# martinmodrak/math

Hardware: AMD Instinct MI355X
Metric: gradient evals/sec (fp64), GP-marginal log-density N=4096 (higher is better)
Workload: dtype f64; 1 GPU; gp_marginal_gradient; N=4096, kernel=exp_quad, parallelism=replicas1

## Files before the change

### include/smg_hip.h

```cpp
#ifndef SMG_HIP_H
#define SMG_HIP_H

#include <stddef.h>

#ifdef __cplusplus
extern "C" {
#endif

enum smg_status_code {
  SMG_OK = 0,
  SMG_ERR_HIP = 1,
  SMG_ERR_NOT_PD = 2,
  SMG_ERR_NOT_SYMMETRIC = 4,
  SMG_ERR_NONFINITE = 8,
  SMG_ERR_ARG = 16,
  SMG_ERR_OOM = 32,
  SMG_ERR_NOT_POSITIVE = 64,
  SMG_ERR_SYNC = 128
};

typedef struct smg_ctx smg_ctx;

int smg_device_count(int* n_host);
int smg_ctx_create(int device, size_t initial_arena_bytes, smg_ctx** out_host);
int smg_ctx_destroy(smg_ctx* ctx);
int smg_ctx_device(const smg_ctx* ctx);
void* smg_ctx_stream(smg_ctx* ctx);

void* smg_arena_alloc(smg_ctx* ctx, size_t bytes);
size_t smg_arena_mark(smg_ctx* ctx);
int smg_arena_rewind(smg_ctx* ctx, size_t mark);
int smg_arena_recover_all(smg_ctx* ctx);
size_t smg_arena_used(const smg_ctx* ctx);
size_t smg_arena_reserved(const smg_ctx* ctx);
void* smg_host_scratch(smg_ctx* ctx, size_t bytes);
void* smg_pinned_io(smg_ctx* ctx, size_t bytes);
void* smg_pinned_result(smg_ctx* ctx, size_t bytes);
int smg_publish_to_host(smg_ctx* ctx, const double* src, long long n, double* dst);
int smg_gather_scalars(smg_ctx* ctx, const double* const* src, int n, double* dst, int* status_out);

int smg_memcpy_h2d(smg_ctx* ctx, void* dst, const void* src_host, size_t bytes);
int smg_memcpy_d2h(smg_ctx* ctx, void* dst_host, const void* src, size_t bytes);
int smg_memcpy_d2d(smg_ctx* ctx, void* dst, const void* src, size_t bytes);
int smg_memset(smg_ctx* ctx, void* dst, int value, size_t bytes);
int smg_memset_async(smg_ctx* ctx, void* dst, size_t bytes);
int smg_join_async(smg_ctx* ctx);
int smg_sync(smg_ctx* ctx);
int smg_sync_all(smg_ctx* ctx);
int smg_marker_record(smg_ctx* ctx, int slot);
int smg_marker_wait(smg_ctx* ctx, int slot);
int smg_status(smg_ctx* ctx, int* status_host);
int smg_status_armed(smg_ctx* ctx, int* armed);
int smg_status_enqueue(smg_ctx* ctx, int* host_dst);
int smg_status_inject(smg_ctx* ctx, int bits);
int smg_set_inv_block_mode(smg_ctx* ctx, int mode);
int smg_inv_block_fused(smg_ctx* ctx, int n);

enum smg_family {
  SMG_FAM_GEMM = 0, SMG_FAM_CHOL_FWD = 1, SMG_FAM_CHOL_REV = 2,
  SMG_FAM_GP = 3, SMG_FAM_MVN = 4, SMG_FAM_TRSV = 5, SMG_FAM_GLM = 6,
  SMG_FAM_ELEMWISE = 7,
  SMG_FAM_PANEL = 8,
  SMG_FAM_COMM = 9,
  SMG_FAM_COUNT = 10
};
int smg_profile_enable(smg_ctx* ctx, int on);
int smg_profile_read(smg_ctx* ctx, int family, double* total_ms_host, long long* count_host);
int smg_profile_flops(smg_ctx* ctx, int family, double* flops_host);

int smg_fill_unif(smg_ctx* ctx, double* out, long long n, unsigned long long seed,
                  double a, double b, double scale);
int smg_fill_bernoulli(smg_ctx* ctx, int* out, long long n, unsigned long long seed, double p);

int smg_gemm(smg_ctx* ctx, int transA, int transB, int uplo, int m, int n, int k,
             double alpha, const double* A, int lda, const double* B, int ldb,
             double beta, double* C, int ldc);
#define SMG_TRI_A_LOWER 1
#define SMG_TRI_A_UPPER 2
#define SMG_TRI_B_LOWER 4
#define SMG_TRI_B_UPPER 8
int smg_gemm_tri(smg_ctx* ctx, int transA, int transB, int uplo, int tri, int m, int n, int k, double alpha,
                 const double* A, int lda, const double* B, int ldb, double beta, double* C, int ldc);


int smg_gp_exp_quad_cov_fwd(smg_ctx* ctx, const double* x, int n, double sigma,
                            double l, double* K, int ldk);
int smg_gp_exp_quad_cov_rev(smg_ctx* ctx, const double* x, int n, double sigma,
                            double l, const double* Kadj, int ldka, double* out2);

int smg_gp_exp_quad_cov_nd_fwd(smg_ctx* ctx, const double* x, int D, int n, double sigma,
                               double l, double* K, int ldk);
int smg_gp_exp_quad_cov_nd_rev(smg_ctx* ctx, const double* x, int D, int n, double sigma,
                               double l, const double* Kadj, int ldka, double* out2);

enum smg_gp_family { SMG_GP_EXP_QUAD = 0, SMG_GP_EXPONENTIAL = 1, SMG_GP_MATERN32 = 2, SMG_GP_MATERN52 = 3 };
int smg_gp_cov_fwd(smg_ctx* ctx, int family, const double* x, int D, int n, double sigma, double l,
                   double* K, int ldk);
int smg_gp_cov_rev(smg_ctx* ctx, int family, const double* x, int D, int n, double sigma, double l,
                   const double* Kadj, int ldka, double* out2);

int smg_gp_exp_quad_cov_tangent_fwd(smg_ctx* ctx, const double* x, int n, double sigma,
                                    double l, double dsigma, double dl, double* Kd, int ldk);
int smg_gp_exp_quad_cov_tangent_rev(smg_ctx* ctx, const double* x, int n, double sigma,
                                    double l, double dsigma, double dl, const double* Kdadj,
                                    int ldka, double* out4);

int smg_add_diag_fwd(smg_ctx* ctx, const double* A, int lda, int n,
                     double d_scalar, const double* d_vec, double* B, int ldb);
int smg_add_diag_rev(smg_ctx* ctx, const double* Badj, int ldb, int n,
                     double* Aadj, int ldaa, double* dadj, int d_is_vec);

long long smg_cholesky_aux_doubles(int n);
int smg_cholesky_block_size(int n);
int smg_check_symmetric(smg_ctx* ctx, const double* A, int lda, int n);
int smg_cholesky_fwd(smg_ctx* ctx, const double* A, int lda, int n, double* L,
// ... 228 lines not shown
```

### math_amd/csrc/ctx.hip

```cpp
#include <cstdio>
#include <cstdlib>
#include <cstring>

#include "smg_internal.h"

namespace {

constexpr size_t kAlign = 256;

__global__ void k_reduce_partials(const double* __restrict__ p, int nparts,
                                  int width, double* out, int accumulate) {
  __shared__ double lds[16];
  const int c = blockIdx.x;
  double s = 0.0;
  for (int i = threadIdx.x; i < nparts; i += blockDim.x) s += p[(size_t)i * width + c];
  s = block_sum(s, lds);
  if (threadIdx.x == 0) out[c] = accumulate ? out[c] + s : s;
}

__global__ __launch_bounds__(256) void k_publish(const double* __restrict__ src, long long n, double* dst,
                                                 long long* done, long long seq) {
  for (long long i = threadIdx.x; i < n; i += blockDim.x)
    __hip_atomic_store(dst + i, src[i], __ATOMIC_RELAXED, __HIP_MEMORY_SCOPE_SYSTEM);
  asm volatile("s_waitcnt vmcnt(0)" ::: "memory");
// ... 198 lines not shown
  ctx->side = nullptr;
  ctx->main_stream = nullptr;
  for (int i = 0; i < SMG_FAM_COUNT; ++i) {
    ctx->prof_ms[i] = 0;
    ctx->prof_count[i] = 0;
    ctx->prof_flops[i] = 0;
  }
  int prio_least = 0, prio_greatest = 0;
  if (hipDeviceGetStreamPriorityRange(&prio_least, &prio_greatest) != hipSuccess) prio_greatest = 0;
  if (hipStreamCreateWithPriority(&ctx->stream, hipStreamNonBlocking, prio_greatest) != hipSuccess) {
    delete ctx;
    return SMG_ERR_HIP;
  }
  if (initial < (size_t)(64u << 20)) initial = (size_t)(64u << 20);
  char* base = nullptr;
  if (hipMalloc(&base, initial) != hipSuccess) {
    hipStreamDestroy(ctx->stream);
    delete ctx;
    return SMG_ERR_OOM;
  }
  ctx->blocks.push_back({base, initial});
  if (hipMalloc(&ctx->status_d, SMG_STATUS_BYTES) != hipSuccess ||
      hipHostMalloc(&ctx->status_h, 256, hipHostMallocDefault) != hipSuccess) {
    delete ctx;
    return SMG_ERR_HIP;
  }
  hipMemset(ctx->status_d, 0, SMG_STATUS_BYTES);
  ctx->flags_d = ctx->status_d + 64;
  ctx->flag_epoch = 0;
  ctx->inv_ctr_d = reinterpret_cast<unsigned*>(ctx->flags_d + 4096);
  ctx->inv_launches = 0;
  ctx->inv_per_cu = ctx->inv_cus = -1;
  ctx->inv_mode = 0;
  ctx->host_scratch_size = 1u << 20;
  if (hipHostMalloc(&ctx->host_scratch, ctx->host_scratch_size, hipHostMallocDefault) != hipSuccess) {
    delete ctx;
    return SMG_ERR_HIP;
  }
  if (hipHostMalloc(&ctx->done_h, 256, hipHostMallocCoherent | hipHostMallocMapped) != hipSuccess ||
      hipMalloc(&ctx->red_counter_d, 256) != hipSuccess) {
    delete ctx;
    return SMG_ERR_HIP;
  }
  *(volatile long long*)ctx->done_h = 0;
  hipMemset(ctx->red_counter_d, 0, 256);
  hipDeviceSynchronize();
  *out = ctx;
  return SMG_OK;
}

int smg_ctx_destroy(smg_ctx* ctx) {
  if (!ctx) return SMG_OK;
  hipSetDevice(ctx->device);
  hipStreamSynchronize(ctx->stream);
  prof_drain(ctx);
  smg_comm_destroy(ctx);
  for (auto& b : ctx->blocks) hipFree(b.base);
  for (auto e : ctx->prof_pool) hipEventDestroy(e);
  for (auto e : ctx->ev_pool) hipEventDestroy(e);
  for (auto e : ctx->ev_fork) hipEventDestroy(e);
  for (auto e : ctx->marker_ev) hipEventDestroy(e);
  if (ctx->status_ev) hipEventDestroy(ctx->status_ev);
  if (ctx->zero_stream) {
    hipStreamSynchronize(ctx->zero_stream);
    hipEventDestroy(ctx->zero_ev_main);
    hipEventDestroy(ctx->zero_ev_done);
// ... 324 lines not shown
int smg_join_async(smg_ctx* ctx) {
  if (!ctx) return SMG_ERR_ARG;
  if (ctx->inv_pending) {
    SMG_HIP_TRY(hipStreamWaitEvent(ctx->stream, ctx->inv_ev, 0));
    ctx->inv_pending = 0;
  }
  if (int e = smg_zero_flush(ctx)) return e;
  if (!ctx->zero_pending) return SMG_OK;
  SMG_HIP_TRY(hipStreamWaitEvent(ctx->stream, ctx->zero_ev_done, 0));
  ctx->zero_pending = 0;
  return SMG_OK;
}

int smg_marker_record(smg_ctx* ctx, int slot) {
  if (!ctx) return SMG_ERR_ARG;
  hipEvent_t e;
  if (int rc = smg_marker_event(ctx, slot, &e)) return rc;
  SMG_HIP_TRY(hipEventRecord(e, ctx->stream));
  return SMG_OK;
}

int smg_marker_wait(smg_ctx* ctx, int slot) {
  if (!ctx || slot < 0 || slot >= (int)ctx->marker_ev.size()) return SMG_ERR_ARG;
  SMG_HIP_TRY(hipEventSynchronize(ctx->marker_ev[slot]));
  return SMG_OK;
}

int smg_set_inv_block_mode(smg_ctx* ctx, int mode) {
  if (!ctx || mode < 0 || mode > 1) return SMG_ERR_ARG;
  ctx->inv_mode = mode;
  return SMG_OK;
}

int smg_sync_all(smg_ctx* ctx) {
  if (!ctx) return SMG_ERR_ARG;
  sync_all_streams(ctx);
  SMG_HIP_TRY(hipGetLastError());
  if (ctx->prof_on) prof_drain(ctx);
  return SMG_OK;
}

int smg_sync(smg_ctx* ctx) {
  SMG_HIP_TRY(hipStreamSynchronize(ctx->stream));
  if (ctx->prof_on) prof_drain(ctx);
  return SMG_OK;
}

int smg_status(smg_ctx* ctx, int* status) {
  hipLaunchKernelGGL(k_status_take, dim3(1), dim3(64), 0, ctx->stream, ctx->status_d, ctx->status_h);
  SMG_LAUNCH_CHECK();
  SMG_HIP_TRY(hipStreamSynchronize(ctx->stream));
  if (ctx->prof_on) prof_drain(ctx);
  int s = ctx->status_h[0] | ctx->host_status;
  ctx->host_status = 0;
  ctx->status_armed = 0;
  if (status) *status = s;
  return SMG_OK;
}

}

int smg_status_mark_impl(smg_ctx* ctx) {
  if (!ctx->status_ev && hipEventCreateWithFlags(&ctx->status_ev, hipEventDisableTiming) != hipSuccess) {
    ctx->status_ev = nullptr;
    return SMG_ERR_HIP;
  }
// ... 127 lines not shown
```

### math_amd/csrc/gemm.hip

```cpp
#include "smg_internal.h"
#include <cstdio>
#include <cstdlib>
#include <type_traits>

#ifndef SMG_GEMM_TRI128_MIN
#define SMG_GEMM_TRI128_MIN 1024
#endif
#ifndef SMG_GEMM_KS2_MAX
#define SMG_GEMM_KS2_MAX 1536
#endif
#ifndef SMG_GEMM_NR64
#define SMG_GEMM_NR64 2
#endif
#ifndef SMG_GEMM_NR32
#define SMG_GEMM_NR32 2
#endif

namespace {

template <int BM, int BK, bool KCONTIG>
struct lds_layout;
template <int BM, int BK>
struct lds_layout<BM, BK, false> {
  static_assert(BM % 32 == 0, "BM");
  static constexpr int size = BK * BM;
  __device__ static int at(int i, int kk) { return kk * BM + (i ^ ((kk & 1) << 4)); }
};
template <int BM, int BK>
struct lds_layout<BM, BK, true> {
  static_assert(BK == 16 || BK == 32, "BK");
  static constexpr int size = BM * BK;
  __device__ static int at(int i, int kk) {
    return i * BK + (kk ^ (BK == 16 ? (i & 14) : ((i & 15) << 1)));
  }
};

template <int I, int N, typename F>
__device__ __forceinline__ void smg_static_for_impl(F&& f) {
  if constexpr (I < N) {
    f(std::integral_constant<int, I>{});
    smg_static_for_impl<I + 1, N>(f);
  }
}
template <int N, typename F>
__device__ __forceinline__ void smg_static_for(F&& f) {
  smg_static_for_impl<0, N>(f);
}

__device__ double g_gemm_zero[2] = {0.0, 0.0};

template <int BM, int BK, bool KCONTIG, int NT = 256>
__device__ __forceinline__ void load_tile(const double* __restrict__ X, int ld,
                                          int rows, int k, int i0, int k0,
                                          double (&r)[BM * BK / NT]) {
  constexpr int PER = BM * BK / NT;
#pragma unroll
  for (int q = 0; q < PER; ++q) {
    const int e = threadIdx.x + NT * q;
    int i, kk;
    if (KCONTIG) {
      i = e / BK;
      kk = e % BK;
    } else {
      kk = e / BM;
      i = e % BM;
    }
    const int gi = i0 + i, gk = k0 + kk;
    const double* p = KCONTIG ? X + ((size_t)gi * ld + gk) : X + (gi + (size_t)gk * ld);
// ... 18 lines not shown
    lds[lds_layout<BM, BK, KCONTIG>::at(i, kk)] = r[q];
  }
}

__device__ __forceinline__ void tri_decode(int t, int& bi, int& bj) {
  int r = (int)((sqrt(8.0 * (double)t + 1.0) - 1.0) * 0.5);
  while ((r + 1) * (r + 2) / 2 <= t) ++r;
  while (r * (r + 1) / 2 > t) --r;
  bi = r;
  bj = t - r * (r + 1) / 2;
}

__device__ __forceinline__ void tri_decode_grouped(int t, int T, int& bi, int& bj) {
  constexpr int G = 8;
  int r, c;
  tri_decode(t, r, c);
  const int r0 = r / G * G, r1 = min(r0 + G, T), h = r1 - r0;
  int q = t - r0 * (r0 + 1) / 2;
  if (q < r0 * h) {
    bi = r0 + q % h;
    bj = q / h;
    return;
  }
  q -= r0 * h;
  int j = r0;
  while (q >= r1 - j) {
    q -= r1 - j;
    ++j;
  }
  bi = j + q;
  bj = j;
}

template <int BM, int BN, int BK, bool TA, bool TB, int MODE, int KS = 1>
__global__ __launch_bounds__(256 * KS) void k_gemm(
    int m, int n, int k, double alpha, const double* __restrict__ A, int lda,
    const double* __restrict__ B, int ldb, double beta, double* __restrict__ C,
    int ldc, int tiles_m, int ntiles, int kchunk, double* __restrict__ slab, long long sA,
    long long sB, long long sC, int px, int ntp, int tri, double* __restrict__ C2, int ldc2, int bz) {
  constexpr bool LOWT = MODE == 1 || MODE == 3;
  constexpr bool UPT = MODE == 2;
  constexpr bool TRIC = LOWT || UPT;
  A += blockIdx.y * sA;
  B += blockIdx.y * sB;
  C += blockIdx.y * sC;
  constexpr bool AK = TA;
  constexpr bool BKC = !TB;
  using LA = lds_layout<BM, BK, AK>;
  using LB = lds_layout<BN, BK, BKC>;
  constexpr int NR = BM == 128 ? 1 : (BM == 64 ? SMG_GEMM_NR64 : SMG_GEMM_NR32);
  constexpr int STAGE = LA::size + LB::size;
  constexpr int OPS = 2 * STAGE;
  constexpr int ECH = (BM * BN + BN <= OPS) ? BN : 32;
  constexpr int POOL = (OPS > (BM + 1) * ECH) ? OPS : (BM + 1) * ECH;
  __shared__ double pool[POOL];

  int bi, bj, tile, split;
  const bool tri_a_only = !TRIC && (tri & 3) && !(tri & 12);
  const bool tri_b_only = !TRIC && (tri & 12) && !(tri & 3);
  if (px > 0) {
    split = blockIdx.x / ntp;
    const int tb = blockIdx.x - split * ntp;
    const int x = tb & 7, l = tb >> 3, py = 8 / px;
    const int tiles_n = ntiles / tiles_m;
    const int rx = x % px, ry = x / px;
    const int r0 = rx * tiles_m / px, r1 = (rx + 1) * tiles_m / px;
    const int c0 = ry * tiles_n / py, c1 = (ry + 1) * tiles_n / py;
    const int rm = r1 - r0;
    if (rm <= 0 || l >= rm * (c1 - c0)) return;
    tile = (r0 + l % rm) + (c0 + l / rm) * tiles_m;
  } else {
    tile = blockIdx.x % ntiles;
    split = blockIdx.x / ntiles;
  }
  const bool tri_sq = TRIC && m == n && BM == BN;
  if (LOWT && tri_sq) {
    const int T = tiles_m;
    int r, q;
    if (tri == SMG_TRI_B_LOWER) {
      tri_decode(ntiles - 1 - tile, r, q);
      bj = T - 1 - r;
      bi = bj + q;
    } else if (tri == SMG_TRI_B_UPPER || tri == (SMG_TRI_A_LOWER | SMG_TRI_B_UPPER)) {
      tri_decode(tile, r, q);
      bj = T - 1 - r;
// ... 32 lines not shown
  if (tri) {
    int lo = 0, hi = k;
    if (tri & 1) hi = min(hi, i0 + BM);
    if (tri & 2) lo = max(lo, i0);
    if (tri & 4) lo = max(lo, j0);
    if (tri & 8) hi = min(hi, j0 + BN);
    lo = lo / BK * BK;
    kbeg = max(kbeg, lo);
    kend = min(kend, hi);
    if (kend < kbeg) kend = kbeg;
  }

  constexpr int TM = BM / 32, TN = BN / 32;
  constexpr int NT = 256 * KS;
  const int lane = threadIdx.x & 63, wave = threadIdx.x >> 6;
  const int wr = (wave & 3) >> 1, wc = wave & 1, kg = KS == 1 ? 0 : wave >> 2;
  d4 acc[TM][TN];
#pragma unroll
  for (int a = 0; a < TM; ++a)
#pragma unroll
    for (int b = 0; b < TN; ++b) acc[a][b] = d4{0.0, 0.0, 0.0, 0.0};

  constexpr int PA = BM * BK / NT, PB = BN * BK / NT;
  double ra[NR][PA], rb[NR][PB];
  const int nst = (kend - kbeg + BK - 1) / BK;
  auto gload = [&](int set, int st) {
    load_tile<BM, BK, AK, NT>(A, lda, m, kend, i0, kbeg + st * BK, ra[set]);
    load_tile<BN, BK, BKC, NT>(B, ldb, n, kend, j0, kbeg + st * BK, rb[set]);
  };
  auto lstore = [&](int set, int buf) {
    store_tile<BM, BK, AK, NT>(pool + buf * STAGE, ra[set]);
    store_tile<BN, BK, BKC, NT>(pool + buf * STAGE + LA::size, rb[set]);
  };
#pragma unroll
  for (int j = 0; j < NR; ++j) gload(j, j);
  constexpr int EPT = BM * BN / NT;
  constexpr bool PREFETCH_C = EPT <= 16;
  const bool use_c = !slab && beta != 0.0 && !(bz > 0 && i0 >= bz) && !(bz < 0 && j0 >= -bz);
  double cpre[PREFETCH_C ? EPT : 1];
  if (PREFETCH_C) {
#pragma unroll
    for (int q = 0; q < EPT; ++q) {
      const int e = threadIdx.x + NT * q;
      const int i = i0 + e % BM, j = j0 + e / BM;
      cpre[q] = (use_c && i < m && j < n) ? C[i + (size_t)j * ldc] : 0.0;
    }
  }
  const int fr = lane & 15, fk = lane >> 4;
  static_assert(BK / 4 % KS == 0, "K stage split");
  auto mma_stage = [&](const double* Ab, const double* Bb) {
#pragma unroll
    for (int kq = 0; kq < BK / 4 / KS; ++kq) {
      const int ks = kg * (BK / 4 / KS) + kq;
      double af[TM], bf[TN];
#pragma unroll
      for (int a = 0; a < TM; ++a)
        af[a] = Ab[LA::at(wr * (BM / 2) + a * 16 + fr, ks * 4 + fk)];
#pragma unroll
      for (int b = 0; b < TN; ++b)
        bf[b] = Bb[LB::at(wc * (BN / 2) + b * 16 + fr, ks * 4 + fk)];
#pragma unroll
      for (int a = 0; a < TM; ++a)
#pragma unroll
        for (int b = 0; b < TN; ++b)
          acc[a][b] = __builtin_amdgcn_mfma_f64_16x16x4f64(af[a], bf[b], acc[a][b], 0, 0, 0);
    }
  };
  lstore(0, 0);
  gload(0, NR);
  __syncthreads();
  constexpr int U = NR % 2 == 0 ? NR : 2 * NR;
  auto body = [&](int st, auto uc) {
    constexpr int u = decltype(uc)::value;
    mma_stage(pool + (u & 1) * STAGE, pool + (u & 1) * STAGE + LA::size);
    lstore((u + 1) % NR, (u & 1) ^ 1);
    gload((u + 1) % NR, st + 1 + NR);
    __syncthreads();
  };
  int s0 = 0;
  for (; s0 + U <= nst; s0 += U)
    smg_static_for<U>([&](auto uc) { body(s0 + decltype(uc)::value, uc); });
  smg_static_for<U - 1>([&](auto uc) {
    if (s0 + decltype(uc)::value < nst) body(s0 + decltype(uc)::value, uc);
  });

  __syncthreads();
#pragma unroll
  for (int c0 = 0; c0 < BN; c0 += ECH) {
#pragma unroll
    for (int g = 0; g < KS; ++g) {
      if (kg == g) {
#pragma unroll
        for (int a = 0; a < TM; ++a)
#pragma unroll
          for (int b = 0; b < TN; ++b) {
            const int jl = wc * (BN / 2) + b * 16 + (lane & 15) - c0;
            if (jl < 0 || jl >= ECH) continue;
#pragma unroll
            for (int r = 0; r < 4; ++r) {
              double* d = &pool[jl * (BM + 1) + wr * (BM / 2) + a * 16 + (lane >> 4) + 4 * r];
              *d = g == 0 ? acc[a][b][r] : *d + acc[a][b][r];
            }
          }
      }
      __syncthreads();
    }
#pragma unroll
    for (int q = 0; q < BM * ECH / NT; ++q) {
      const int e = threadIdx.x + NT * q;
      const int il = e % BM, jl = e / BM;
      const int i = i0 + il, j = j0 + c0 + jl;
      if (i >= m || j >= n) continue;
      if (LOWT && i < j) {
        if (MODE == 3 && C2) C2[i + (size_t)j * ldc2] = 0.0;
        continue;
      }
      if (UPT && i > j) continue;
// ... 38 lines not shown
                                                        double alpha, double beta, double* __restrict__ C, int ldc,
                                                        int lower, int bz) {
  const long long tot = (long long)m * n;
  for (smg_mn w(m >> 1, n); w.ok(); w.next()) {
    const int i = 2 * w.i, j = w.j;
    if (lower == 1 && i + 1 < j) continue;
    if (lower == 2 && i > j) continue;
    const long long e = (long long)j * m + i;
    d2v s = {0.0, 0.0};
    int t = 0;
    for (; t + 4 <= splits; t += 4) {
      const d2v a0 = *reinterpret_cast<const d2v*>(slab + (size_t)t * tot + e);
      const d2v a1 = *reinterpret_cast<const d2v*>(slab + (size_t)(t + 1) * tot + e);
      const d2v a2 = *reinterpret_cast<const d2v*>(slab + (size_t)(t + 2) * tot + e);
      const d2v a3 = *reinterpret_cast<const d2v*>(slab + (size_t)(t + 3) * tot + e);
      s += a0;
      s += a1;
      s += a2;
      s += a3;
    }
    for (; t < splits; ++t) s += *reinterpret_cast<const d2v*>(slab + (size_t)t * tot + e);
    double* c = C + i + (size_t)j * ldc;
    const bool w0 = !(lower == 1 && i < j), w1 = !(lower == 2 && i + 1 > j);
    const double b = ((bz > 0 && i >= bz) || (bz < 0 && j >= -bz)) ? 0.0 : beta;
    if (w0) c[0] = (b == 0.0) ? alpha * s[0] : alpha * s[0] + b * c[0];
    if (w1) c[1] = (b == 0.0) ? alpha * s[1] : alpha * s[1] + b * c[1];
  }
}

thread_local double* t_c2 = nullptr;
thread_local int t_ldc2 = 0;
thread_local int t_bz = 0;

template <int BM, int BN, int BK, bool TA, bool TB, int MODE, int KS = 1>
int launch(smg_ctx* ctx, int m, int n, int k, double alpha, const double* A,
           int lda, const double* B, int ldb, double beta, double* C, int ldc, int batch = 1,
           long long sA = 0, long long sB = 0, long long sC = 0, int tri = 0) {
  constexpr bool TRIC = MODE == 1 || MODE == 2 || MODE == 3;
  const int tm = smg_ceil_div(m, BM), tn = smg_ceil_div(n, BN);
  const int ntiles = (TRIC && m == n && BM == BN) ? tm * (tm + 1) / 2 : tm * tn;
  int splits = 1;
  const int target = 512;
  constexpr int KMIN = 64;
  const bool covers = ntiles >= 256 && k <= 1024;
  if (!tri && MODE != 3 && MODE != 4 && batch == 1 && ntiles < target && !covers &&
      k >= 2 * KMIN) {
    splits = smg_ceil_div(target, ntiles);
    const int maxs = k / KMIN;
    if (splits > maxs) splits = maxs;
    if (splits > 64) splits = 64;
    if (splits < 1) splits = 1;
  }
  int kchunk = smg_ceil_div(smg_ceil_div(k, splits), BK) * BK;
  splits = smg_ceil_div(k, kchunk);
  double* slab = nullptr;
  if (splits > 1) {
    const int slot = ctx->stream == ctx->side                                ? SMG_WS_GEMM_SIDE
                     : (ctx->zero_stream && ctx->stream == ctx->zero_stream) ? SMG_WS_GEMM_ZERO
                                                                             : SMG_WS_GEMM;
    slab = smg_ws(ctx, slot, (size_t)splits * m * n);
    if (!slab) return SMG_ERR_OOM;
  }
  const bool tri_one = !TRIC && tri && (!(tri & 3) || !(tri & 12));
  int px = 0, ntp = ntiles;
  if (!(TRIC && m == n && BM == BN) && ntiles >= 64 && !tri_one) {
    long long best = -1;
    for (int p = 1; p <= 8; p *= 2) {
      const int q = 8 / p;
      if (p > tm || q > tn) continue;
      const long long rr = smg_ceil_div(tm, p), cc = smg_ceil_div(tn, q);
      const long long foot = rr * BM + cc * BN;
      if (best < 0 || foot < best) {
        best = foot;
        px = p;
        ntp = 8 * (int)(rr * cc);
      }
    }
  }
  hipLaunchKernelGGL((k_gemm<BM, BN, BK, TA, TB, MODE, KS>), dim3(ntp * splits, batch), dim3(256 * KS), 0,
                     ctx->stream, m, n, k, alpha, A, lda, B, ldb, beta, C, ldc, tm,
                     ntiles, kchunk, slab, sA, sB, sC, px, ntp, tri, MODE >= 3 ? t_c2 : nullptr,
                     MODE >= 3 ? t_ldc2 : 0, t_bz);
  if (splits > 1) {
    const long long tot = (long long)m * n;
    if ((m & 1) == 0) {
      const long long pairs = tot / 2;
      const int nb = (int)(pairs / 256 < 2048 ? (pairs + 255) / 256 : 2048);
      hipLaunchKernelGGL(k_splitk_reduce2, dim3(nb), dim3(256), 0, ctx->stream, m, n, splits, slab, alpha, beta,
                         C, ldc, MODE, t_bz);
    } else {
      hipLaunchKernelGGL(k_splitk_reduce, dim3(smg_ceil_div(tot, 256)), dim3(256), 0,
                         ctx->stream, m, n, splits, slab, alpha, beta, C, ldc, MODE, t_bz);
    }
  }
  SMG_LAUNCH_CHECK();
  return SMG_OK;
}

inline bool overlaps(const double* X, int ldx, int rows, int cols, const double* C, int ldc, int m,
                     int n) {
  if (rows <= 0 || cols <= 0 || m <= 0 || n <= 0) return false;
  const double* x1 = X + (size_t)(cols - 1) * ldx + rows;
  const double* c1 = C + (size_t)(n - 1) * ldc + m;
  if (!(X < c1 && C < x1)) return false;
  if (ldx != ldc) return true;
  const double* base = X < C ? X : C;
  const long long ox = X - base, oc = C - base, ld = ldx;
  const long long rx = ox % ld, cx = ox / ld, rc = oc % ld, cc = oc / ld;
  return rx < rc + m && rc < rx + rows && cx < cc + n && cc < cx + cols;
}

constexpr int BK64 = 16;

template <bool TA, bool TB, int MODE>
int dispatch_tile(smg_ctx* ctx, int m, int n, int k, double alpha, const double* A,
                  int lda, const double* B, int ldb, double beta, double* C, int ldc, int tri) {
  constexpr bool FULLC = MODE == 0 || MODE == 4;
  const bool alias_a = overlaps(A, lda, TA ? k : m, TA ? m : k, C, ldc, m, n);
  const bool alias_b = overlaps(B, ldb, TB ? n : k, TB ? k : n, C, ldc, m, n);
  if (alias_a || alias_b) {
    if (MODE == 3 || MODE == 4 || t_bz) return SMG_ERR_ARG;
    if (MODE == 0 && alias_a && !alias_b && n <= 64)
      return launch<32, 64, 32, TA, TB, 0>(ctx, m, n, k, alpha, A, lda, B, ldb, beta, C, ldc, 1, 0, 0, 0, tri);
    if (MODE == 0 && alias_b && !alias_a && m <= 64)
      return launch<64, 32, 32, TA, TB, 0>(ctx, m, n, k, alpha, A, lda, B, ldb, beta, C, ldc, 1, 0, 0, 0, tri);
    double* T = smg_ws(ctx, SMG_WS_ALIAS, (size_t)m * n);
    if (!T) return SMG_ERR_OOM;
    int rc = dispatch_tile<TA, TB, MODE>(ctx, m, n, k, alpha, A, lda, B, ldb, 0.0, T, m, tri);
    if (rc) return rc;
    if (beta == 0.0) return smg_copy_impl(ctx, m, n, T, m, C, ldc, 1.0, 0);
    if (beta != 1.0) {
      rc = smg_scale_impl(ctx, m, n, beta, C, ldc, MODE);
      if (rc) return rc;
    }
    return smg_copy_impl(ctx, m, n, T, m, C, ldc, 1.0, 1);
  }
  const long long big_tiles = (long long)smg_ceil_div(m, 128) * smg_ceil_div(n, 128);
  const long long t64 = smg_ceil_div(m, 64);
  const long long mid_tiles =
      (!FULLC && m == n) ? t64 * (t64 + 1) / 2 : t64 * smg_ceil_div(n, 64);
  if (FULLC && big_tiles >= (tri ? SMG_GEMM_TRI128_MIN : 256) && k > 128)
    return launch<128, 128, 16, TA, TB, MODE>(ctx, m, n, k, alpha, A, lda, B, ldb, beta, C, ldc, 1, 0, 0, 0, tri);
  if (MODE == 0 && TA && !TB && k >= 1536 && mid_tiles < 512)
    return launch<128, 64, 16, TA, TB, MODE>(ctx, m, n, k, alpha, A, lda, B, ldb, beta, C, ldc, 1, 0, 0, 0, tri);
  if (mid_tiles >= 512) {
    if (mid_tiles <= SMG_GEMM_KS2_MAX)
      return launch<64, 64, BK64, TA, TB, MODE, 2>(ctx, m, n, k, alpha, A, lda, B, ldb, beta, C, ldc, 1, 0, 0, 0, tri);
    return launch<64, 64, BK64, TA, TB, MODE>(ctx, m, n, k, alpha, A, lda, B, ldb, beta, C, ldc, 1, 0, 0, 0, tri);
  }
  const bool tall_nn = MODE == 0 && !TA && !TB && n <= 512;
  if (mid_tiles >= 256 && !tall_nn)
    return launch<64, 64, BK64, TA, TB, MODE, 2>(ctx, m, n, k, alpha, A, lda, B, ldb, beta, C, ldc, 1, 0, 0, 0, tri);
  const long long t32 = smg_ceil_div(m, 32);
  const long long small_tiles = (!FULLC && m == n) ? t32 * (t32 + 1) / 2 : t32 * smg_ceil_div(n, 32);
  if (small_tiles <= 256)
    return launch<32, 32, 32, TA, TB, MODE, 2>(ctx, m, n, k, alpha, A, lda, B, ldb, beta, C, ldc, 1, 0, 0, 0, tri);
  return launch<32, 32, 32, TA, TB, MODE>(ctx, m, n, k, alpha, A, lda, B, ldb, beta, C, ldc, 1, 0, 0, 0, tri);
}

}

int smg_gemm_batched_impl(smg_ctx* ctx, int ta, int tb, int m, int n, int k, double alpha,
                          const double* A, int lda, long long sA, const double* B, int ldb,
                          long long sB, double beta, double* C, int ldc, long long sC, int batch) {
  if (m <= 0 || n <= 0 || batch <= 0) return SMG_OK;
  if (k <= 0 || alpha == 0.0) return SMG_ERR_ARG;
  smg_prof_scope prof(ctx, SMG_FAM_GEMM);
  if (ctx->prof_on) ctx->prof_flops[SMG_FAM_GEMM] += 2.0 * m * n * k * batch;
  const bool big = (long long)smg_ceil_div(m, 64) * smg_ceil_div(n, 64) * batch >= 192;
#define SMG_BATCHED(TA_, TB_)                                                                    \
  return big ? launch<64, 64, BK64, TA_, TB_, 0>(ctx, m, n, k, alpha, A, lda, B, ldb, beta, C, ldc, \
                                               batch, sA, sB, sC)                                 \
             : launch<32, 32, 32, TA_, TB_, 0>(ctx, m, n, k, alpha, A, lda, B, ldb, beta, C, ldc, \
// ... 71 lines not shown

int smg_gemm_sym_phi_impl(smg_ctx* ctx, int ta, int tb, int n, int k, double alpha, const double* A, int lda,
                          const double* B, int ldb, double beta, double* C, int ldc, double* P, int ldp, int tri) {
  if (n <= 0) return SMG_OK;
  if (k <= 0 || alpha == 0.0 || !P) return SMG_ERR_ARG;
  smg_prof_scope prof(ctx, SMG_FAM_GEMM);
  if (ctx->prof_on) {
    const double cut = (tri & 3) && (tri & 12) ? 1.0 / 3.0 : (tri ? 0.5 : 1.0);
    ctx->prof_flops[SMG_FAM_GEMM] += cut * 2.0 * k * ((double)n * n - (double)n * (n - 1) / 2);
  }
  t_c2 = P;
  t_ldc2 = ldp;
  int rc;
  if (!ta && !tb) rc = dispatch_tile<false, false, 3>(ctx, n, n, k, alpha, A, lda, B, ldb, beta, C, ldc, tri);
  else if (ta && !tb) rc = dispatch_tile<true, false, 3>(ctx, n, n, k, alpha, A, lda, B, ldb, beta, C, ldc, tri);
  else if (!ta && tb) rc = dispatch_tile<false, true, 3>(ctx, n, n, k, alpha, A, lda, B, ldb, beta, C, ldc, tri);
  else rc = dispatch_tile<true, true, 3>(ctx, n, n, k, alpha, A, lda, B, ldb, beta, C, ldc, tri);
  t_c2 = nullptr;
  return rc;
}

extern "C" int smg_gemm_tri(smg_ctx* ctx, int ta, int tb, int uplo, int tri, int m, int n, int k,
                            double alpha, const double* A, int lda, const double* B, int ldb, double beta,
                            double* C, int ldc) {
  if (!ctx || m < 0 || n < 0 || k < 0 || tri < 0 || tri > 15) return SMG_ERR_ARG;
  if ((m > 0 && n > 0) && (!C || ldc < m)) return SMG_ERR_ARG;
  if (k > 0 && m > 0 && n > 0 && alpha != 0.0) {
    if (!A || !B) return SMG_ERR_ARG;
    if (lda < (ta ? k : m) || ldb < (tb ? n : k)) return SMG_ERR_ARG;
  }
  return smg_gemm_impl(ctx, ta, tb, uplo, m, n, k, alpha, A, lda, B, ldb, beta, C, ldc, tri);
}

extern "C" int smg_gemm(smg_ctx* ctx, int ta, int tb, int uplo, int m, int n, int k,
                        double alpha, const double* A, int lda, const double* B,
                        int ldb, double beta, double* C, int ldc) {
  if (!ctx || m < 0 || n < 0 || k < 0) return SMG_ERR_ARG;
  if ((m > 0 && n > 0) && (!C || ldc < m)) return SMG_ERR_ARG;
  if (k > 0 && m > 0 && n > 0 && alpha != 0.0) {
    if (!A || !B) return SMG_ERR_ARG;
    if (lda < (ta ? k : m) || ldb < (tb ? n : k)) return SMG_ERR_ARG;
  }
  return smg_gemm_impl(ctx, ta, tb, uplo, m, n, k, alpha, A, lda, B, ldb, beta, C, ldc);
}
```

### math_amd/csrc/smg_internal.h

```cpp
#pragma once
#include <hip/hip_runtime.h>

#include <cstddef>
#include <cstdint>
#include <utility>
#include <vector>

#include "../../include/smg_hip.h"

typedef double d4 __attribute__((ext_vector_type(4)));
typedef double d2v __attribute__((ext_vector_type(2)));

struct smg_arena_block {
  char* base;
  size_t size;
};

struct smg_prof_slot {
  hipEvent_t start, stop;
  int family;
};

constexpr int SMG_INV_CTRS = 64;
constexpr size_t SMG_STATUS_BYTES = 256 + 4096 * sizeof(int) + SMG_INV_CTRS * sizeof(int);

struct smg_ctx {
  int device;
  hipStream_t stream;
  hipStream_t side;
  hipStream_t main_stream;
  std::vector<hipEvent_t> ev_pool;
  std::vector<hipEvent_t> ev_fork;
  std::vector<hipEvent_t> marker_ev;
  std::vector<smg_arena_block> blocks;
  size_t cur_block;
  size_t offset;
  int* status_d;
  int* status_h;
  int host_status;
  int status_armed;
  hipEvent_t status_ev;
  int status_mark;
  hipStream_t zero_stream;
  hipStream_t copy_stream;
  hipEvent_t zero_ev_main, zero_ev_done;
  int zero_pending;
  std::vector<std::pair<void*, size_t>> zero_queue;
  hipEvent_t inv_ev, inv_ev_main, inv_ev_aux;
  int inv_pending;
  hipEvent_t inv_ev_w;
  int inv_w_recorded;
  int* flags_d;
  int flag_epoch;
  unsigned* inv_ctr_d;
  long long inv_launches;
  int inv_per_cu, inv_cus;
  int inv_mode;
  void* host_scratch;
  size_t host_scratch_size;
  void* pin_io;
  size_t pin_io_size;
  void* res_h;
  size_t res_h_size;
  long long* done_h;
  long long done_seq;
  unsigned int* red_counter_d;
  double* ws[12];
  size_t ws_doubles[12];
  int prof_on;
  std::vector<smg_prof_slot> prof_pending;
  std::vector<hipEvent_t> prof_pool;
  double prof_ms[SMG_FAM_COUNT];
  double prof_flops[SMG_FAM_COUNT];
  long long prof_count[SMG_FAM_COUNT];
  void* comm;
};

#define SMG_HIP_TRY(expr)                          \
  do {                                             \
    hipError_t _e = (expr);                        \
    if (_e != hipSuccess) {                        \
      if (ctx) ctx->host_status |= SMG_ERR_HIP;    \
      return SMG_ERR_HIP;                          \
    }                                              \
  } while (0)

#define SMG_LAUNCH_CHECK()                         \
  do {                                             \
    hipError_t _e = hipGetLastError();             \
    if (_e != hipSuccess) {                        \
// ... 138 lines not shown
```

### math_amd/hip.py

```python
import ctypes
import os

import numpy as np

_HERE = os.path.dirname(os.path.abspath(__file__))
LIB_PATH = os.path.join(_HERE, "lib", "libsmg_hip.so")

SMG_OK = 0
STATUS = {1: "hip", 2: "not_pd", 4: "not_symmetric", 8: "nonfinite", 16: "arg", 32: "oom", 64: "not_positive"}
GP_FAMILIES = {"exp_quad": 0, "exponential": 1, "matern32": 2, "matern52": 3}
FAMILIES = {"gemm": 0, "chol_fwd": 1, "chol_rev": 2, "gp": 3, "mvn": 4, "trsv": 5, "glm": 6, "elementwise": 7, "panel": 8, "comm": 9}

_P = ctypes.c_void_p
_I = ctypes.c_int
_L = ctypes.c_longlong
_D = ctypes.c_double
_S = ctypes.c_size_t

_SIGS = {
    "smg_device_count": (_I, [ctypes.POINTER(_I)]),
    "smg_ctx_create": (_I, [_I, _S, ctypes.POINTER(_P)]),
    "smg_ctx_destroy": (_I, [_P]),
    "smg_ctx_device": (_I, [_P]),
    "smg_ctx_stream": (_P, [_P]),
    "smg_arena_alloc": (_P, [_P, _S]),
    "smg_arena_mark": (_S, [_P]),
    "smg_arena_rewind": (_I, [_P, _S]),
    "smg_arena_recover_all": (_I, [_P]),
    "smg_arena_used": (_S, [_P]),
    "smg_arena_reserved": (_S, [_P]),
    "smg_host_scratch": (_P, [_P, _S]),
    "smg_memcpy_h2d": (_I, [_P, _P, _P, _S]),
    "smg_memcpy_d2h": (_I, [_P, _P, _P, _S]),
    "smg_memcpy_d2d": (_I, [_P, _P, _P, _S]),
    "smg_memset": (_I, [_P, _P, _I, _S]),
    "smg_memset_async": (_I, [_P, _P, _S]),
    "smg_join_async": (_I, [_P]),
    "smg_sync": (_I, [_P]),
    "smg_sync_all": (_I, [_P]),
    "smg_status": (_I, [_P, ctypes.POINTER(_I)]),
    "smg_status_armed": (_I, [_P, ctypes.POINTER(_I)]),
    "smg_status_enqueue": (_I, [_P, _P]),
    "smg_status_inject": (_I, [_P, _I]),
    "smg_set_inv_block_mode": (_I, [_P, _I]),
    "smg_inv_block_fused": (_I, [_P, _I]),
    "smg_pinned_io": (_P, [_P, _S]),
    "smg_pinned_result": (_P, [_P, _S]),
    "smg_gather_scalars": (_I, [_P, _P, _I, _P, _P]),
    "smg_pack_tril": (_I, [_P, _I, _I, _P, _I, _P]),
    "smg_unpack_tril_add": (_I, [_P, _I, _I, _P, _P, _I]),
    "smg_publish_to_host": (_I, [_P, _P, _L, _P]),
    "smg_profile_enable": (_I, [_P, _I]),
    "smg_profile_read": (_I, [_P, _I, ctypes.POINTER(_D), ctypes.POINTER(_L)]),
    "smg_profile_flops": (_I, [_P, _I, ctypes.POINTER(_D)]),
    "smg_fill_unif": (_I, [_P, _P, _L, ctypes.c_ulonglong, _D, _D, _D]),
    "smg_fill_bernoulli": (_I, [_P, _P, _L, ctypes.c_ulonglong, _D]),
    "smg_gemm": (_I, [_P, _I, _I, _I, _I, _I, _I, _D, _P, _I, _P, _I, _D, _P, _I]),
    "smg_gemm_tri": (_I, [_P, _I, _I, _I, _I, _I, _I, _I, _D, _P, _I, _P, _I, _D, _P, _I]),
    "smg_gp_exp_quad_cov_fwd": (_I, [_P, _P, _I, _D, _D, _P, _I]),
    "smg_gp_exp_quad_cov_rev": (_I, [_P, _P, _I, _D, _D, _P, _I, _P]),
    "smg_bernoulli_logit_glm_checked": (_I, [_P, _P, _P, _L, _I, _L, _P, _P, _P]),
    "smg_bernoulli_logit_glm_io": (_I, [_P, _P, _P, _L, _I, _L, _D, _P, _P, _P, _P]),
    "smg_marker_record": (_I, [_P, _I]),
    "smg_marker_wait": (_I, [_P, _I]),
    "smg_gp_exp_quad_cov_nd_fwd": (_I, [_P, _P, _I, _I, _D, _D, _P, _I]),
    "smg_gp_exp_quad_cov_nd_rev": (_I, [_P, _P, _I, _I, _D, _D, _P, _I, _P]),
    "smg_add_diag_fwd": (_I, [_P, _P, _I, _I, _D, _P, _P, _I]),
    "smg_add_diag_rev": (_I, [_P, _P, _I, _I, _P, _I, _P, _I]),
    "smg_cholesky_block_size": (_I, [_I]),
    "smg_check_symmetric": (_I, [_P, _P, _I, _I]),
    "smg_cholesky_fwd": (_I, [_P, _P, _I, _I, _P, _I, _P]),
    "smg_cholesky_fwd_checked": (_I, [_P, _P, _I, _I, _P, _I, _P]),
    "smg_cholesky_fwd_checked_mark": (_I, [_P, _P, _I, _I, _P, _I, _P]),
    "smg_status_mark_wait": (_I, [_P, _P]),
    "smg_cholesky_rev": (_I, [_P, _P, _I, _P, _P, _I, _I, _P, _I]),
    "smg_mdivide_left_tri_fwd": (_I, [_P, _I, _P, _I, _P, _I, _I, _I, _P, _I]),
    "smg_mdivide_left_tri_rev": (_I, [_P, _I, _P, _I, _P, _I, _P, _I, _I, _I, _P, _I, _P, _I, _P]),
    "smg_mdivide_left_tri_aux_fwd": (_I, [_P, _I, _P, _I, _P, _P, _I, _I, _I, _P, _I]),
    "smg_mdivide_left_tri_aux_rev": (_I, [_P, _I, _P, _I, _P, _P, _I, _P, _I, _I, _I, _P, _I, _P, _I, _P]),
    "smg_chol_tangent_fwd": (_I, [_P, _P, _I, _P, _P, _I, _I, _P, _P, _P, _P, _P, _I]),
    "smg_chol_tangent_fwd_w": (_I, [_P, _P, _I, _P, _P, _I, _I, _P, _P, _P, _P, _I]),
    "smg_chol_tangent_rev": (_I, [_P, _P, _I, _P, _P, _P, _P, _I, _P, _I, _I, _P, _I, _P, _I, _P]),
    "smg_multiply_lower_fwd": (_I, [_P, _P, _I, _P, _I, _I, _P, _I]),
    "smg_multiply_lower_rev": (_I, [_P, _P, _I, _P, _I, _P, _I, _I, _P, _I, _P, _I, _P]),
    "smg_multiply_fwd": (_I, [_P, _P, _I, _P, _I, _I, _I, _I, _P, _I]),
    "smg_multiply_rev": (_I, [_P, _P, _I, _P, _I, _P, _I, _I, _I, _I, _P, _I, _P, _I]),
    "smg_mvn_cholesky_fwd": (_I, [_P, _P, _P, _P, _I, _P, _I, _P, _P]),
    "smg_mvn_cholesky_rev": (_I, [_P, _P, _I, _P, _I, _P, _D, _I, _P, _P, _P, _I]),
    "smg_mvn_cholesky_fwd_inv": (_I, [_P, _P, _P, _P, _I, _P, _I, _I, _P, _P]),
    "smg_cholesky_inverse_wait": (_I, [_P]),
    "smg_cholesky_inverse_adjoint": (_I, [_P, _P, _I, _I, _P, _I, _L, _D, _P, _I]),
# ... 196 lines not shown
```

Baseline: 406.1 gradient evals/s.

## Stage GEMM operand tiles via direct global-to-LDS DMA with multi-buffering

Adds a 64x64 GEMM variant that loads A and B tiles straight into LDS with global_load_lds_dwordx4 instead of going through registers, keeping two or three stage buffers in flight with waitcnt-plus-barrier synchronisation. A dispatch policy picks this path for mid-sized tiles with k >= 512 on aligned, evenly divisible shapes, and disables split-k for it. The aim is to cut register pressure and the LDS store instructions on the mid-size GEMMs used by the Cholesky and GP gradient, and to overlap loads with MFMA work. In exchange it relies on inline assembly with m0 manipulation and hand-derived swizzle inverses, and it drops split-k parallelism for these shapes. It also exposes a mode setter and a smg_gemm_bz entry point.

```diff
diff --git a/include/smg_hip.h b/include/smg_hip.h
--- a/include/smg_hip.h
+++ b/include/smg_hip.h
@@ -55,6 +55,7 @@
 int smg_status_inject(smg_ctx* ctx, int bits);
 int smg_set_inv_block_mode(smg_ctx* ctx, int mode);
 int smg_inv_block_fused(smg_ctx* ctx, int n);
+int smg_set_gemm_stage_mode(smg_ctx* ctx, int mode);
 
 enum smg_family {
   SMG_FAM_GEMM = 0, SMG_FAM_CHOL_FWD = 1, SMG_FAM_CHOL_REV = 2,
@@ -81,6 +82,8 @@
 #define SMG_TRI_B_UPPER 8
 int smg_gemm_tri(smg_ctx* ctx, int transA, int transB, int uplo, int tri, int m, int n, int k, double alpha,
                  const double* A, int lda, const double* B, int ldb, double beta, double* C, int ldc);
+int smg_gemm_bz(smg_ctx* ctx, int transA, int transB, int uplo, int tri, int m, int n, int k, double alpha,
+                const double* A, int lda, const double* B, int ldb, double beta, double* C, int ldc, int bz);
 
 
 int smg_gp_exp_quad_cov_fwd(smg_ctx* ctx, const double* x, int n, double sigma,
diff --git a/math_amd/csrc/ctx.hip b/math_amd/csrc/ctx.hip
--- a/math_amd/csrc/ctx.hip
+++ b/math_amd/csrc/ctx.hip
@@ -254,6 +254,7 @@
   ctx->inv_launches = 0;
   ctx->inv_per_cu = ctx->inv_cus = -1;
   ctx->inv_mode = 0;
+  ctx->gemm_stage = 0;
   ctx->host_scratch_size = 1u << 20;
   if (hipHostMalloc(&ctx->host_scratch, ctx->host_scratch_size, hipHostMallocDefault) != hipSuccess) {
     delete ctx;
@@ -644,6 +645,12 @@
   return SMG_OK;
 }
 
+int smg_set_gemm_stage_mode(smg_ctx* ctx, int mode) {
+  if (!ctx || mode < 0 || mode > 2) return SMG_ERR_ARG;
+  ctx->gemm_stage = mode;
+  return SMG_OK;
+}
+
 int smg_sync_all(smg_ctx* ctx) {
   if (!ctx) return SMG_ERR_ARG;
   sync_all_streams(ctx);
diff --git a/math_amd/csrc/gemm.hip b/math_amd/csrc/gemm.hip
--- a/math_amd/csrc/gemm.hip
+++ b/math_amd/csrc/gemm.hip
@@ -8,6 +8,27 @@
 #endif
 #ifndef SMG_GEMM_KS2_MAX
 #define SMG_GEMM_KS2_MAX 1536
+#endif
+#ifndef SMG_GEMM_DMA_BK1
+#define SMG_GEMM_DMA_BK1 16
+#endif
+#ifndef SMG_GEMM_DMA_NB1
+#define SMG_GEMM_DMA_NB1 3
+#endif
+#ifndef SMG_GEMM_DMA_BK2
+#define SMG_GEMM_DMA_BK2 32
+#endif
+#ifndef SMG_GEMM_DMA_NB2
+#define SMG_GEMM_DMA_NB2 2
+#endif
+#ifndef SMG_GEMM_DMA_KS2_MAX
+#define SMG_GEMM_DMA_KS2_MAX 512
+#endif
+#ifndef SMG_GEMM_DMA_MIN_TILES
+#define SMG_GEMM_DMA_MIN_TILES 136
+#endif
+#ifndef SMG_GEMM_DMA_FAMILIES
+#define SMG_GEMM_DMA_FAMILIES 31
 #endif
 #ifndef SMG_GEMM_NR64
 #define SMG_GEMM_NR64 2
@@ -25,6 +46,10 @@
   static_assert(BM % 32 == 0, "BM");
   static constexpr int size = BK * BM;
   __device__ static int at(int i, int kk) { return kk * BM + (i ^ ((kk & 1) << 4)); }
+  __device__ static void from(int p, int& i, int& kk) {
+    kk = p / BM;
+    i = (p % BM) ^ ((kk & 1) << 4);
+  }
 };
 template <int BM, int BK>
 struct lds_layout<BM, BK, true> {
@@ -33,7 +58,27 @@
   __device__ static int at(int i, int kk) {
     return i * BK + (kk ^ (BK == 16 ? (i & 14) : ((i & 15) << 1)));
   }
+  __device__ static void from(int p, int& i, int& kk) {
+    i = p / BK;
+    kk = (p % BK) ^ (BK == 16 ? (i & 14) : ((i & 15) << 1));
+  }
 };
+
+__device__ __forceinline__ void dma16(const double* g, unsigned lds) {
+  unsigned keep;
+  asm volatile(
+      "s_mov_b32 %0, m0\n\ts_mov_b32 m0, %2\n\ts_nop 0\n\tglobal_load_lds_dwordx4 %1, off\n\ts_mov_b32 m0, %0"
+      : "=&s"(keep)
+      : "v"(g), "s"(lds)
+      : "memory");
+}
+
+template <int N>
+__device__ __forceinline__ void dma_wait_barrier() {
+  asm volatile("s_waitcnt vmcnt(%0) lgkmcnt(0)" ::"n"(N) : "memory");
+  __builtin_amdgcn_s_barrier();
+  asm volatile("" ::: "memory");
+}
 
 template <int I, int N, typename F>
 __device__ __forceinline__ void smg_static_for_impl(F&& f) {
@@ -118,7 +163,7 @@
   bj = j;
 }
 
-template <int BM, int BN, int BK, bool TA, bool TB, int MODE, int KS = 1>
+template <int BM, int BN, int BK, bool TA, bool TB, int MODE, int KS = 1, int NB = 0>
 __global__ __launch_bounds__(256 * KS) void k_gemm(
     int m, int n, int k, double alpha, const double* __restrict__ A, int lda,
     const double* __restrict__ B, int ldb, double beta, double* __restrict__ C,
@@ -136,7 +181,7 @@
   using LB = lds_layout<BN, BK, BKC>;
   constexpr int NR = BM == 128 ? 1 : (BM == 64 ? SMG_GEMM_NR64 : SMG_GEMM_NR32);
   constexpr int STAGE = LA::size + LB::size;
-  constexpr int OPS = 2 * STAGE;
+  constexpr int OPS = (NB ? NB : 2) * STAGE;
   constexpr int ECH = (BM * BN + BN <= OPS) ? BN : 32;
   constexpr int POOL = (OPS > (BM + 1) * ECH) ? OPS : (BM + 1) * ECH;
   __shared__ double pool[POOL];
@@ -235,8 +280,10 @@
     store_tile<BM, BK, AK, NT>(pool + buf * STAGE, ra[set]);
     store_tile<BN, BK, BKC, NT>(pool + buf * STAGE + LA::size, rb[set]);
   };
-#pragma unroll
-  for (int j = 0; j < NR; ++j) gload(j, j);
+  if constexpr (NB == 0) {
+#pragma unroll
+    for (int j = 0; j < NR; ++j) gload(j, j);
+  }
   constexpr int EPT = BM * BN / NT;
   constexpr bool PREFETCH_C = EPT <= 16;
   const bool use_c = !slab && beta != 0.0 && !(bz > 0 && i0 >= bz) && !(bz < 0 && j0 >= -bz);
@@ -269,6 +316,7 @@
           acc[a][b] = __builtin_amdgcn_mfma_f64_16x16x4f64(af[a], bf[b], acc[a][b], 0, 0, 0);
     }
   };
+  if constexpr (NB == 0) {
   lstore(0, 0);
   gload(0, NR);
   __syncthreads();
@@ -286,6 +334,55 @@
   smg_static_for<U - 1>([&](auto uc) {
     if (s0 + decltype(uc)::value < nst) body(s0 + decltype(uc)::value, uc);
   });
+  } else {
+    constexpr int NW = 4 * KS;
+    constexpr int QA = BK / 2 / NW;
+    constexpr int L = 2 * QA;
+    static_assert(BM == 64 && BN == 64 && BK / 2 % NW == 0 && (NB == 2 || NB == 3), "DMA staging: 64 x 64 tile");
+    static_assert(AK ? (128 * NW / BK) % 16 == 0 : true, "DMA staging: swizzle period");
+    static_assert(NB * STAGE * 8 <= 65536, "DMA staging: LDS");
+    const int wv = __builtin_amdgcn_readfirstlane(wave);
+    const double *pa, *pb;
+    {
+      int i, kk;
+      LA::from(wv * 128 + 2 * lane, i, kk);
+      pa = AK ? A + ((size_t)(i0 + i) * lda + kbeg + kk) : A + ((i0 + i) + (size_t)(kbeg + kk) * lda);
+      LB::from(wv * 128 + 2 * lane, i, kk);
+      pb = BKC ? B + ((size_t)(j0 + i) * ldb + kbeg + kk) : B + ((j0 + i) + (size_t)(kbeg + kk) * ldb);
+    }
+    const long long qsa = (long long)(AK ? 128 * NW / BK : 2 * NW) * lda;
+    const long long qsb = (long long)(BKC ? 128 * NW / BK : 2 * NW) * ldb;
+    const long long ssa = AK ? BK : (long long)BK * lda, ssb = BKC ? BK : (long long)BK * ldb;
+    const unsigned ldsw = (unsigned)(size_t)pool + wv * 1024;
+    auto issue = [&](auto bc) {
+      constexpr int buf = decltype(bc)::value;
+#pragma unroll
+      for (int q = 0; q < QA; ++q) dma16(pa + q * qsa, ldsw + (buf * STAGE) * 8 + q * NW * 1024);
+#pragma unroll
+      for (int q = 0; q < QA; ++q) dma16(pb + q * qsb, ldsw + (buf * STAGE + LA::size) * 8 + q * NW * 1024);
+      pa += ssa;
+      pb += ssb;
+    };
+    auto step = [&](int st, auto uc, auto full) {
+      constexpr int u = decltype(uc)::value;
+      constexpr bool FULL = decltype(full)::value;
+      if (NB == 3 && (FULL || st + 1 < nst)) dma_wait_barrier<L>();
+      else dma_wait_barrier<0>();
+      if (FULL || st + NB - 1 < nst) issue(std::integral_constant<int, (u + NB - 1) % NB>{});
+      mma_stage(pool + u * STAGE, pool + u * STAGE + LA::size);
+    };
+    if (nst > 0) {
+      issue(std::integral_constant<int, 0>{});
+      if (NB == 3 && nst > 1) issue(std::integral_constant<int, 1>{});
+      int s0 = 0;
+      for (; s0 + 2 * NB - 1 <= nst; s0 += NB)
+        smg_static_for<NB>([&](auto uc) { step(s0 + decltype(uc)::value, uc, std::true_type{}); });
+      for (; s0 < nst; s0 += NB)
+        smg_static_for<NB>([&](auto uc) {
+          if (s0 + decltype(uc)::value < nst) step(s0 + decltype(uc)::value, uc, std::false_type{});
+        });
+    }
+  }
 
   __syncthreads();
 #pragma unroll
@@ -390,7 +487,7 @@
 thread_local int t_ldc2 = 0;
 thread_local int t_bz = 0;
 
-template <int BM, int BN, int BK, bool TA, bool TB, int MODE, int KS = 1>
+template <int BM, int BN, int BK, bool TA, bool TB, int MODE, int KS = 1, int NB = 0>
 int launch(smg_ctx* ctx, int m, int n, int k, double alpha, const double* A,
            int lda, const double* B, int ldb, double beta, double* C, int ldc, int batch = 1,
            long long sA = 0, long long sB = 0, long long sC = 0, int tri = 0) {
@@ -401,7 +498,7 @@
   const int target = 512;
   constexpr int KMIN = 64;
   const bool covers = ntiles >= 256 && k <= 1024;
-  if (!tri && MODE != 3 && MODE != 4 && batch == 1 && ntiles < target && !covers &&
+  if (NB == 0 && !tri && MODE != 3 && MODE != 4 && batch == 1 && ntiles < target && !covers &&
       k >= 2 * KMIN) {
     splits = smg_ceil_div(target, ntiles);
     const int maxs = k / KMIN;
@@ -435,7 +532,7 @@
       }
     }
   }
-  hipLaunchKernelGGL((k_gemm<BM, BN, BK, TA, TB, MODE, KS>), dim3(ntp * splits, batch), dim3(256 * KS), 0,
+  hipLaunchKernelGGL((k_gemm<BM, BN, BK, TA, TB, MODE, KS, NB>), dim3(ntp * splits, batch), dim3(256 * KS), 0,
                      ctx->stream, m, n, k, alpha, A, lda, B, ldb, beta, C, ldc, tm,
                      ntiles, kchunk, slab, sA, sB, sC, px, ntp, tri, MODE >= 3 ? t_c2 : nullptr,
                      MODE >= 3 ? t_ldc2 : 0, t_bz);
@@ -470,9 +567,17 @@
 
 constexpr int BK64 = 16;
 
+inline bool dma_eligible(int m, int n, int k, const double* A, int lda, const double* B, int ldb,
+                         const double* C, int ldc) {
+  constexpr int KQ = SMG_GEMM_DMA_BK1 > SMG_GEMM_DMA_BK2 ? SMG_GEMM_DMA_BK1 : SMG_GEMM_DMA_BK2;
+  return m % 64 == 0 && n % 64 == 0 && k > 0 && k % KQ == 0 && !((lda | ldb | ldc) & 1) &&
+         !(((size_t)A | (size_t)B | (size_t)C) & 15);
+}
+
 template <bool TA, bool TB, int MODE>
 int dispatch_tile(smg_ctx* ctx, int m, int n, int k, double alpha, const double* A,
-                  int lda, const double* B, int ldb, double beta, double* C, int ldc, int tri) {
+                  int lda, const double* B, int ldb, double beta, double* C, int ldc, int tri,
+                  bool aliased = false) {
   constexpr bool FULLC = MODE == 0 || MODE == 4;
   const bool alias_a = overlaps(A, lda, TA ? k : m, TA ? m : k, C, ldc, m, n);
   const bool alias_b = overlaps(B, ldb, TB ? n : k, TB ? k : n, C, ldc, m, n);
@@ -484,7 +589,7 @@
       return launch<64, 32, 32, TA, TB, 0>(ctx, m, n, k, alpha, A, lda, B, ldb, beta, C, ldc, 1, 0, 0, 0, tri);
     double* T = smg_ws(ctx, SMG_WS_ALIAS, (size_t)m * n);
     if (!T) return SMG_ERR_OOM;
-    int rc = dispatch_tile<TA, TB, MODE>(ctx, m, n, k, alpha, A, lda, B, ldb, 0.0, T, m, tri);
+    int rc = dispatch_tile<TA, TB, MODE>(ctx, m, n, k, alpha, A, lda, B, ldb, 0.0, T, m, tri, true);
     if (rc) return rc;
     if (beta == 0.0) return smg_copy_impl(ctx, m, n, T, m, C, ldc, 1.0, 0);
     if (beta != 1.0) {
@@ -497,6 +602,21 @@
   const long long t64 = smg_ceil_div(m, 64);
   const long long mid_tiles =
       (!FULLC && m == n) ? t64 * (t64 + 1) / 2 : t64 * smg_ceil_div(n, 64);
+  if constexpr (MODE == 0 || MODE == 1) {
+    constexpr int fam = MODE == 1 ? (!TA && TB ? 1 : TA && !TB ? 2 : !TA && !TB ? 16 : 0)
+                                  : (!TA && !TB ? 4 : TA && !TB ? 8 : 0);
+    const bool g128 = FULLC && big_tiles >= (tri ? SMG_GEMM_TRI128_MIN : 256) && k > 128;
+    const bool policy = (SMG_GEMM_DMA_FAMILIES & fam) && k >= 512 && !(g128 && !tri) &&
+                        (mid_tiles >= 256 || (mid_tiles >= SMG_GEMM_DMA_MIN_TILES && k <= 1024));
+    const bool want = ctx->gemm_stage == 2 || (ctx->gemm_stage == 0 && policy);
+    if (want && !aliased && dma_eligible(m, n, k, A, lda, B, ldb, C, ldc)) {
+      if (mid_tiles <= SMG_GEMM_DMA_KS2_MAX)
+        return launch<64, 64, SMG_GEMM_DMA_BK2, TA, TB, MODE, 2, SMG_GEMM_DMA_NB2>(ctx, m, n, k, alpha, A, lda, B, ldb,
+                                                                                 beta, C, ldc, 1, 0, 0, 0, tri);
+      return launch<64, 64, SMG_GEMM_DMA_BK1, TA, TB, MODE, 1, SMG_GEMM_DMA_NB1>(ctx, m, n, k, alpha, A, lda, B, ldb,
+                                                                               beta, C, ldc, 1, 0, 0, 0, tri);
+    }
+  }
   if (FULLC && big_tiles >= (tri ? SMG_GEMM_TRI128_MIN : 256) && k > 128)
     return launch<128, 128, 16, TA, TB, MODE>(ctx, m, n, k, alpha, A, lda, B, ldb, beta, C, ldc, 1, 0, 0, 0, tri);
   if (MODE == 0 && TA && !TB && k >= 1536 && mid_tiles < 512)
@@ -634,6 +754,14 @@
   return smg_gemm_impl(ctx, ta, tb, uplo, m, n, k, alpha, A, lda, B, ldb, beta, C, ldc, tri);
 }
 
+extern "C" int smg_gemm_bz(smg_ctx* ctx, int ta, int tb, int uplo, int tri, int m, int n, int k, double alpha,
+                           const double* A, int lda, const double* B, int ldb, double beta, double* C, int ldc,
+                           int bz) {
+  if (!ctx || m <= 0 || n <= 0 || k <= 0 || tri < 0 || tri > 15 || alpha == 0.0) return SMG_ERR_ARG;
+  if (!A || !B || !C || ldc < m || lda < (ta ? k : m) || ldb < (tb ? n : k)) return SMG_ERR_ARG;
+  return smg_gemm_bz_impl(ctx, ta, tb, uplo, m, n, k, alpha, A, lda, B, ldb, beta, C, ldc, tri, bz);
+}
+
 extern "C" int smg_gemm(smg_ctx* ctx, int ta, int tb, int uplo, int m, int n, int k,
                         double alpha, const double* A, int lda, const double* B,
                         int ldb, double beta, double* C, int ldc) {
diff --git a/math_amd/csrc/smg_internal.h b/math_amd/csrc/smg_internal.h
--- a/math_amd/csrc/smg_internal.h
+++ b/math_amd/csrc/smg_internal.h
@@ -56,6 +56,7 @@
   long long inv_launches;
   int inv_per_cu, inv_cus;
   int inv_mode;
+  int gemm_stage;
   void* host_scratch;
   size_t host_scratch_size;
   void* pin_io;
diff --git a/math_amd/hip.py b/math_amd/hip.py
--- a/math_amd/hip.py
+++ b/math_amd/hip.py
@@ -44,6 +44,7 @@
     "smg_status_inject": (_I, [_P, _I]),
     "smg_set_inv_block_mode": (_I, [_P, _I]),
     "smg_inv_block_fused": (_I, [_P, _I]),
+    "smg_set_gemm_stage_mode": (_I, [_P, _I]),
     "smg_pinned_io": (_P, [_P, _S]),
     "smg_pinned_result": (_P, [_P, _S]),
     "smg_gather_scalars": (_I, [_P, _P, _I, _P, _P]),
@@ -57,6 +58,7 @@
     "smg_fill_bernoulli": (_I, [_P, _P, _L, ctypes.c_ulonglong, _D]),
     "smg_gemm": (_I, [_P, _I, _I, _I, _I, _I, _I, _D, _P, _I, _P, _I, _D, _P, _I]),
     "smg_gemm_tri": (_I, [_P, _I, _I, _I, _I, _I, _I, _I, _D, _P, _I, _P, _I, _D, _P, _I]),
+    "smg_gemm_bz": (_I, [_P, _I, _I, _I, _I, _I, _I, _I, _D, _P, _I, _P, _I, _D, _P, _I, _I]),
     "smg_gp_exp_quad_cov_fwd": (_I, [_P, _P, _I, _D, _D, _P, _I]),
     "smg_gp_exp_quad_cov_rev": (_I, [_P, _P, _I, _D, _D, _P, _I, _P]),
     "smg_bernoulli_logit_glm_checked": (_I, [_P, _P, _P, _L, _I, _L, _P, _P, _P]),
```

Result: faster. 460.3 gradient evals/s (median of 6 runs) (+13.4%).
